# ygjwd12345/UCD

Measured on AMD Instinct MI355X. Metric: images/sec (whole node) per UCD train step, VOC 15-5 step-1, 513^2 bs=24, higher is better.
Workload: dtype bf16

## Files before the change

ucd_amd/csrc/stem.hip:

```cpp
#include "common.h"

namespace ucd {
namespace {

typedef __hip_bfloat16 bf16;
constexpr int kThreads = 256;
constexpr int kRedBlocks = 1024;
constexpr int kApplyRows = 4;

__device__ __forceinline__ float leaky(float z, float slope) { return z > 0.f ? z : z * slope; }
__device__ __forceinline__ float bf16_round(float v) { return __bfloat162float(__float2bfloat16(v)); }

struct StemArgs {
  const bf16* z; int B, H, W, C, PH, PW;
  const float *mean, *scale, *beta, *invstd, *weight, *sums;
  float slope, inv_count;
  int abs_gamma, cg_shift;
};

__global__ __launch_bounds__(kThreads) void stem_apply_pool_kernel(StemArgs p, bf16* __restrict__ out, uint8_t* __restrict__ idx) {
  const int cgs = p.cg_shift, CG = 1 << cgs;
  const int t = blockIdx.x * kThreads + threadIdx.x;
  const int cg = t & (CG - 1), pw = t >> cgs, ph = blockIdx.y, b = blockIdx.z;
  if (pw >= p.PW) return;
  const size_t pix = ((size_t)b * p.PH + ph) * p.PW + pw;
  float mu[8], sc[8], sh[8], best[8];
  int bi[8];
#pragma unroll
  for (int e = 0; e < 8; ++e) {
    mu[e] = p.mean[cg * 8 + e]; sc[e] = p.scale[cg * 8 + e]; sh[e] = p.beta ? p.beta[cg * 8 + e] : 0.f;
    best[e] = -INFINITY; bi[e] = 0;
  }
  Vec<bf16> v[9];
#pragma unroll
  for (int kh = 0; kh < 3; ++kh) {
    const int y = min(max(2 * ph - 1 + kh, 0), p.H - 1);
#pragma unroll
    for (int kw = 0; kw < 3; ++kw) {
      const int x = min(max(2 * pw - 1 + kw, 0), p.W - 1);
      v[kh * 3 + kw].load(p.z + (((size_t)b * p.H + y) * p.W + x) * p.C + cg * 8);
    }
  }
#pragma unroll
  for (int kh = 0; kh < 3; ++kh) {
    const bool yin = (unsigned)(2 * ph - 1 + kh) < (unsigned)p.H;
#pragma unroll
    for (int kw = 0; kw < 3; ++kw) {
      const bool in = yin && (unsigned)(2 * pw - 1 + kw) < (unsigned)p.W;
#pragma unroll
      for (int e = 0; e < 8; ++e) {
        const float a = bf16_round(leaky((v[kh * 3 + kw].get(e) - mu[e]) * sc[e] + sh[e], p.slope));
        if (in && a > best[e]) { best[e] = a; bi[e] = kh * 3 + kw; }
      }
    }
  }
  Vec<bf16> o;
#pragma unroll
  for (int e = 0; e < 8; ++e) o.set(e, best[e]);
  o.store(out + pix * p.C + cg * 8);
  if (idx) {
    uint2 w;
    w.x = (unsigned)bi[0] | ((unsigned)bi[1] << 8) | ((unsigned)bi[2] << 16) | ((unsigned)bi[3] << 24);
    w.y = (unsigned)bi[4] | ((unsigned)bi[5] << 8) | ((unsigned)bi[6] << 16) | ((unsigned)bi[7] << 24);
    *reinterpret_cast<uint2*>(idx + pix * p.C + cg * 8) = w;
  }
}

__global__ __launch_bounds__(kThreads) void stem_pool_bwd_reduce_kernel(StemArgs p, const bf16* __restrict__ dpool,
                                                                       const uint8_t* __restrict__ idx, float* __restrict__ partial) {
  extern __shared__ __attribute__((aligned(16))) float lds[];
  const int CG = p.C / 8, PL = kThreads / CG;
  const int cg = threadIdx.x % CG, pl = threadIdx.x / CG;
  const long long npix = (long long)p.B * p.PH * p.PW;
  float acc[16];
#pragma unroll
  for (int i = 0; i < 16; ++i) acc[i] = 0.f;
  if (pl < PL) {
    float mu[8], sc[8], sh[8], is[8];
#pragma unroll
    for (int e = 0; e < 8; ++e) {
      mu[e] = p.mean[cg * 8 + e]; sc[e] = p.scale[cg * 8 + e]; sh[e] = p.beta ? p.beta[cg * 8 + e] : 0.f; is[e] = p.invstd[cg * 8 + e];
    }
    for (int pix = blockIdx.x * PL + pl; pix < (int)npix; pix += gridDim.x * PL) {
      const int rowi = pix / p.PW;
      const int pw = pix - rowi * p.PW, b = rowi / p.PH, ph = rowi - b * p.PH;
      Vec<bf16> g;
      g.load(dpool + (size_t)pix * p.C + cg * 8);
      const uint2 w = *reinterpret_cast<const uint2*>(idx + (size_t)pix * p.C + cg * 8);
      float zsel[8] = {0.f, 0.f, 0.f, 0.f, 0.f, 0.f, 0.f, 0.f};
      Vec<bf16> v[9];
#pragma unroll
      for (int kh = 0; kh < 3; ++kh) {
        const int y = min(max(2 * ph - 1 + kh, 0), p.H - 1);
#pragma unroll
        for (int kw = 0; kw < 3; ++kw) {
          const int x = min(max(2 * pw - 1 + kw, 0), p.W - 1);
          v[kh * 3 + kw].load(p.z + (((size_t)b * p.H + y) * p.W + x) * p.C + cg * 8);
        }
      }
#pragma unroll
      for (int pos = 0; pos < 9; ++pos)
#pragma unroll
        for (int e = 0; e < 8; ++e) {
          const unsigned id = ((e < 4 ? w.x : w.y) >> (8 * (e & 3))) & 0xffu;
          zsel[e] = id == (unsigned)pos ? v[pos].get(e) : zsel[e];
        }
#pragma unroll
      for (int e = 0; e < 8; ++e) {
        const float xc = zsel[e] - mu[e];
        const float dz = g.get(e) * (xc * sc[e] + sh[e] > 0.f ? 1.f : p.slope);
        acc[e] += dz;
        acc[8 + e] += dz * (xc * is[e]);
      }
    }
  }
#pragma unroll
  for (int i = 0; i < 16; ++i) lds[threadIdx.x * 16 + i] = acc[i];
  __syncthreads();
  if (pl == 0) {
    for (int l = 1; l < PL; ++l)
#pragma unroll
      for (int i = 0; i < 16; ++i) acc[i] += lds[(l * CG + cg) * 16 + i];
    float* dst = partial + (size_t)blockIdx.x * 2 * p.C + cg * 8;
#pragma unroll
    for (int e = 0; e < 8; ++e) { dst[e] = acc[e]; dst[p.C + e] = acc[8 + e]; }
  }
}

__global__ __launch_bounds__(kThreads) void stem_pool_bwd_apply_kernel(StemArgs p, const bf16* __restrict__ dpool,
                                                                      const uint8_t* __restrict__ idx, bf16* __restrict__ dz) {
  const int cgs = p.cg_shift, CG = 1 << cgs;
  const int t = blockIdx.x * kThreads + threadIdx.x;
  const int cg = t & (CG - 1), i = t >> cgs, b = blockIdx.z;
  if (2 * i >= p.W) return;
  float mu[8], sc[8], sh[8], is[8], k0[8], k1[8], gw[8];
#pragma unroll
  for (int e = 0; e < 8; ++e) {
    const int ch = cg * 8 + e;
    mu[e] = p.mean[ch]; sc[e] = p.scale[ch]; sh[e] = p.beta ? p.beta[ch] : 0.f; is[e] = p.invstd[ch];
    k0[e] = p.sums[ch] * p.inv_count;
    k1[e] = p.sums[p.C + ch] * p.inv_count;
    if (p.abs_gamma) {
      if (p.weight && p.weight[ch] < 0.f) k1[e] = -k1[e];
      gw[e] = sc[e];
    } else {
      gw[e] = (p.weight ? p.weight[ch] : 1.f) * is[e];
    }
  }
  const int phb = blockIdx.y * 2, y0 = blockIdx.y * kApplyRows, x0 = 2 * i;
  Vec<bf16> g[3][2], v[kApplyRows][2];
  uint2 w[3][2];
  bool gv[3][2];
#pragma unroll
  for (int a = 0; a < 3; ++a)
#pragma unroll
    for (int c = 0; c < 2; ++c) {
      gv[a][c] = phb + a < p.PH && i + c < p.PW;
      const size_t off = (((size_t)b * p.PH + min(phb + a, p.PH - 1)) * p.PW + min(i + c, p.PW - 1)) * p.C + cg * 8;
      w[a][c] = *reinterpret_cast<const uint2*>(idx + off);
      g[a][c].load(dpool + off);
    }
#pragma unroll
  for (int r = 0; r < kApplyRows; ++r)
#pragma unroll
    for (int cx = 0; cx < 2; ++cx)
      v[r][cx].load(p.z + (((size_t)b * p.H + min(y0 + r, p.H - 1)) * p.W + min(x0 + cx, p.W - 1)) * p.C + cg * 8);
#pragma unroll
  for (int r = 0; r < kApplyRows; ++r) {
    if (y0 + r >= p.H) break;
#pragma unroll
    for (int cx = 0; cx < 2; ++cx) {
      if (x0 + cx >= p.W) continue;
      float dy[8] = {0.f, 0.f, 0.f, 0.f, 0.f, 0.f, 0.f, 0.f};
#pragma unroll
      for (int ya = 0; ya < 2; ++ya) {
        if (ya == 1 && !(r & 1)) continue;
        const int a = (r >> 1) + ya, kh = (r & 1) ? (ya ? 0 : 2) : 1;
#pragma unroll
        for (int xa = 0; xa < 2; ++xa) {
          if (xa == 1 && !cx) continue;
          const int kw = cx ? (xa ? 0 : 2) : 1;
          const unsigned pos = gv[a][xa] ? (unsigned)(kh * 3 + kw) : 0xffu;
#pragma unroll
          for (int e = 0; e < 8; ++e) {
            const unsigned id = ((e < 4 ? w[a][xa].x : w[a][xa].y) >> (8 * (e & 3))) & 0xffu;
            dy[e] += id == pos ? g[a][xa].get(e) : 0.f;
          }
        }
      }
      Vec<bf16> o;
#pragma unroll
      for (int e = 0; e < 8; ++e) {
        const float xc = v[r][cx].get(e) - mu[e];
        const float dza = dy[e] * (xc * sc[e] + sh[e] > 0.f ? 1.f : p.slope);
        o.set(e, (dza - k0[e] - (xc * is[e]) * k1[e]) * gw[e]);
      }
      o.store(dz + (((size_t)b * p.H + y0 + r) * p.W + x0 + cx) * p.C + cg * 8);
    }
  }
}

__global__ __launch_bounds__(kThreads) void stem_sum_partials_kernel(const float* __restrict__ partial, int rows, int C,
                                                                    const float* __restrict__ sign_of, float* __restrict__ sums) {
  __shared__ float red[kThreads];
  const int k = blockIdx.x;
  float s = 0.f;
  for (int r = threadIdx.x; r < rows; r += kThreads) s += partial[(size_t)r * 2 * C + k];
  red[threadIdx.x] = s;
  __syncthreads();
  for (int st = kThreads / 2; st > 0; st >>= 1) {
    if (threadIdx.x < st) red[threadIdx.x] += red[threadIdx.x + st];
    __syncthreads();
  }
  if (threadIdx.x == 0) {
    float t = red[0];
    if (sign_of && k >= C && sign_of[k - C] < 0.f) t = -t;
    sums[k] = t;
  }
}

constexpr int kSTH = 8, kSTW = 32;
constexpr int kSIR = 2 * kSTH + 5;
constexpr int kSIP = 216;
constexpr int kSWP = 184;
constexpr int kSK = 176;

struct StemConvArgs {
  const float* x; long long sb, sc, sh, sw;
  const bf16* w;
  bf16* z;
  int B, H, W, OH, OW, tiles_y, tiles_x, ntiles;
};

__global__ __launch_bounds__(kThreads) void stem_conv7x7_kernel(StemConvArgs p) {
  typedef float f32x16 __attribute__((ext_vector_type(16)));
  typedef __bf16 bf16x8 __attribute__((ext_vector_type(8)));
  __shared__ __attribute__((aligned(16))) unsigned short Wl[64 * kSWP];
  __shared__ __attribute__((aligned(16))) unsigned short In[kSIR * kSIP];
  const int tid = threadIdx.x, lane = tid & 63, wave = tid >> 6;
  for (int i = tid; i < 64 * kSWP; i += kThreads) Wl[i] = 0;
  __syncthreads();
  for (int i = tid; i < 64 * 147; i += kThreads) {
    const int n = i / 147, r = i - n * 147, ky = r / 21, j = r - ky * 21;
    Wl[n * kSWP + ky * 24 + j] = reinterpret_cast<const unsigned short*>(p.w)[i];
  }
  const int col = lane & 31, h = lane >> 5;
  const int fe = tid < kSIP ? tid : kSIP - 1, fpx = fe / 3, fc = fe - fpx * 3;
  float pre[kSIR];
  unsigned premask = 0;
  auto fetch = [&](int tile) {
    unsigned okm = 0;
    const int b = tile / (p.tiles_y * p.tiles_x), rem = tile - b * p.tiles_y * p.tiles_x;
    const int oy0 = (rem / p.tiles_x) * kSTH, ox0 = (rem % p.tiles_x) * kSTW;
    const int ix = 2 * ox0 - 3 + fpx;
    const bool colok = fpx < 2 * kSTW + 5 && (unsigned)ix < (unsigned)p.W;
    const float* src = p.x + b * p.sb + fc * p.sc + (colok ? ix : 0) * p.sw;
#pragma unroll
    for (int r = 0; r < kSIR; ++r) {
      const int iy = 2 * oy0 - 3 + r;
      const bool ok = colok && (unsigned)iy < (unsigned)p.H;
      const float v = src[(ok ? iy : 0) * p.sh];
      pre[r] = ok ? v : 0.f;
      okm |= 1u << r;
    }
    premask = okm;
  };
  if ((int)blockIdx.x < p.ntiles) fetch(blockIdx.x);
  for (int tile = blockIdx.x; tile < p.ntiles; tile += gridDim.x) {
    const int b = tile / (p.tiles_y * p.tiles_x), rem = tile - b * p.tiles_y * p.tiles_x;
    const int oy0 = (rem / p.tiles_x) * kSTH, ox0 = (rem % p.tiles_x) * kSTW;
    __syncthreads();
    if (tid < kSIP) {
#pragma unroll
      for (int r = 0; r < kSIR; ++r) {
        const bf16 v = __float2bfloat16((premask >> r) & 1u ? pre[r] : 0.f);
        In[r * kSIP + tid] = *reinterpret_cast<const unsigned short*>(&v);
      }
    }
    __syncthreads();
    if (tile + (int)gridDim.x < p.ntiles) fetch(tile + gridDim.x);
    f32x16 acc[2][2];
#pragma unroll
    for (int a = 0; a < 2; ++a)
#pragma unroll
      for (int c = 0; c < 2; ++c)
#pragma unroll
        for (int r = 0; r < 16; ++r) acc[a][c][r] = 0.f;
#pragma unroll
    for (int s = 0; s < kSK / 16; ++s) {
      const int t0 = 2 * s, t1 = 2 * s + 1;
      const int ky = h ? (t1 / 3 > 6 ? 6 : t1 / 3) : t0 / 3, j0 = h ? 8 * (t1 % 3) : 8 * (t0 % 3);
      bf16x8 wf[2], pf[2];
#pragma unroll
      for (int c = 0; c < 2; ++c) wf[c] = *reinterpret_cast<const bf16x8*>(&Wl[(c * 32 + col) * kSWP + 16 * s + 8 * h]);
#pragma unroll
      for (int a = 0; a < 2; ++a) {
        const int orow = wave * 2 + a;
        const unsigned* src = reinterpret_cast<const unsigned*>(&In[(2 * orow + ky) * kSIP + 6 * col + j0]);
        union { unsigned u[4]; bf16x8 v; } f;
        f.u[0] = src[0]; f.u[1] = src[1]; f.u[2] = src[2]; f.u[3] = src[3];
        pf[a] = f.v;
      }
#pragma unroll
      for (int a = 0; a < 2; ++a)
#pragma unroll
        for (int c = 0; c < 2; ++c) acc[a][c] = __builtin_amdgcn_mfma_f32_32x32x16_bf16(wf[c], pf[a], acc[a][c], 0, 0, 0);
    }
    const int ox = ox0 + col;
#pragma unroll
    for (int a = 0; a < 2; ++a) {
      const int oy = oy0 + wave * 2 + a;
      if (oy >= p.OH || ox >= p.OW) continue;
      bf16* dst = p.z + (((size_t)b * p.OH + oy) * p.OW + ox) * 64;
#pragma unroll
      for (int c = 0; c < 2; ++c)
#pragma unroll
        for (int g = 0; g < 4; ++g) {
          union { bf16 v[4]; uint2 u; } o;
#pragma unroll
          for (int e = 0; e < 4; ++e) o.v[e] = __float2bfloat16(acc[a][c][g * 4 + e]);
          *reinterpret_cast<uint2*>(dst + c * 32 + 8 * g + 4 * h) = o.u;
        }
    }
  }
}

constexpr int kFPH = 3, kFPW = 15;
constexpr int kFTP = 72;
struct StemFusedArgs {
  StemConvArgs c;
  const float *mean, *scale, *beta;
  float slope;
  bf16* out;
  int PH, PW;
};

__global__ __launch_bounds__(kThreads) void stem_conv_pool_kernel(StemFusedArgs q) {
  typedef float f32x16 __attribute__((ext_vector_type(16)));
  typedef __bf16 bf16x8 __attribute__((ext_vector_type(8)));
  const StemConvArgs& p = q.c;
  extern __shared__ __attribute__((aligned(16))) unsigned char fs_raw[];
  unsigned short* Wl = reinterpret_cast<unsigned short*>(fs_raw);
  unsigned short* In = Wl + 64 * kSWP;
  unsigned short* Tl = In + kSIR * kSIP;
  float* Pl = reinterpret_cast<float*>(Tl + kSTH * kSTW * kFTP);
  const int tid = threadIdx.x, lane = tid & 63, wave = tid >> 6;
  for (int i = tid; i < 64 * kSWP; i += kThreads) Wl[i] = 0;
  if (tid < 64) { Pl[tid] = q.mean[tid]; Pl[64 + tid] = q.scale[tid]; Pl[128 + tid] = q.beta ? q.beta[tid] : 0.f; }
  __syncthreads();
  for (int i = tid; i < 64 * 147; i += kThreads) {
    const int n = i / 147, r = i - n * 147, ky = r / 21, j = r - ky * 21;
    Wl[n * kSWP + ky * 24 + j] = reinterpret_cast<const unsigned short*>(p.w)[i];
  }
  const int col = lane & 31, h = lane >> 5;
  const int fe = tid < kSIP ? tid : kSIP - 1, fpx = fe / 3, fc = fe - fpx * 3;
  float pre[kSIR];
  unsigned premask = 0;
  auto origin = [&](int tile, int& b, int& oy0, int& ox0) {
    b = tile / (p.tiles_y * p.tiles_x);
    const int rem = tile - b * p.tiles_y * p.tiles_x;
    oy0 = 2 * (rem / p.tiles_x) * kFPH - 1;
    ox0 = 2 * (rem % p.tiles_x) * kFPW - 1;
  };
  auto fetch = [&](int tile) {
    unsigned okm = 0;
    int b, oy0, ox0;
    origin(tile, b, oy0, ox0);
    const int ix = 2 * ox0 - 3 + fpx;
    const bool colok = fpx < 2 * kSTW + 5 && (unsigned)ix < (unsigned)p.W;
    const float* src = p.x + b * p.sb + fc * p.sc + (colok ? ix : 0) * p.sw;
#pragma unroll
    for (int r = 0; r < kSIR; ++r) {
      const int iy = 2 * oy0 - 3 + r;
      const bool ok = colok && (unsigned)iy < (unsigned)p.H;
      pre[r] = src[(ok ? iy : 0) * p.sh];
      okm |= ok ? (1u << r) : 0u;
    }
    premask = okm;
  };
  if ((int)blockIdx.x < p.ntiles) fetch(blockIdx.x);
  for (int tile = blockIdx.x; tile < p.ntiles; tile += gridDim.x) {
    int b, oy0, ox0;
    origin(tile, b, oy0, ox0);
    __syncthreads();
    if (tid < kSIP) {
#pragma unroll
      for (int r = 0; r < kSIR; ++r) {
        const bf16 v = __float2bfloat16((premask >> r) & 1u ? pre[r] : 0.f);
        In[r * kSIP + tid] = *reinterpret_cast<const unsigned short*>(&v);
      }
    }
    __syncthreads();
    if (tile + (int)gridDim.x < p.ntiles) fetch(tile + gridDim.x);
    f32x16 acc[2][2];
#pragma unroll
    for (int a = 0; a < 2; ++a)
#pragma unroll
      for (int c = 0; c < 2; ++c)
#pragma unroll
        for (int r = 0; r < 16; ++r) acc[a][c][r] = 0.f;
#pragma unroll
    for (int s = 0; s < kSK / 16; ++s) {
      const int t0 = 2 * s, t1 = 2 * s + 1;
      const int ky = h ? (t1 / 3 > 6 ? 6 : t1 / 3) : t0 / 3, j0 = h ? 8 * (t1 % 3) : 8 * (t0 % 3);
      bf16x8 wf[2], pf[2];
#pragma unroll
      for (int c = 0; c < 2; ++c) wf[c] = *reinterpret_cast<const bf16x8*>(&Wl[(c * 32 + col) * kSWP + 16 * s + 8 * h]);
#pragma unroll
      for (int a = 0; a < 2; ++a) {
        const int orow = wave * 2 + a;
        const unsigned* src = reinterpret_cast<const unsigned*>(&In[(2 * orow + ky) * kSIP + 6 * col + j0]);
        union { unsigned u[4]; bf16x8 v; } f;
        f.u[0] = src[0]; f.u[1] = src[1]; f.u[2] = src[2]; f.u[3] = src[3];
        pf[a] = f.v;
      }
#pragma unroll
      for (int a = 0; a < 2; ++a)
#pragma unroll
        for (int c = 0; c < 2; ++c) acc[a][c] = __builtin_amdgcn_mfma_f32_32x32x16_bf16(wf[c], pf[a], acc[a][c], 0, 0, 0);
    }
    const int ox = ox0 + col;
#pragma unroll
    for (int a = 0; a < 2; ++a) {
      const int orow = wave * 2 + a, oy = oy0 + orow;
      const bool inside = (unsigned)oy < (unsigned)p.OH && (unsigned)ox < (unsigned)p.OW;
      unsigned short* dst = Tl + (orow * kSTW + col) * kFTP;
#pragma unroll
      for (int c = 0; c < 2; ++c)
#pragma unroll
        for (int g = 0; g < 4; ++g) {
          const int ch = c * 32 + 8 * g + 4 * h;
          const float4 mu = *reinterpret_cast<const float4*>(Pl + ch), sc = *reinterpret_cast<const float4*>(Pl + 64 + ch);
          const float4 sh = *reinterpret_cast<const float4*>(Pl + 128 + ch);
          const float m4[4] = {mu.x, mu.y, mu.z, mu.w}, s4[4] = {sc.x, sc.y, sc.z, sc.w}, b4[4] = {sh.x, sh.y, sh.z, sh.w};
          union { bf16 v[4]; uint2 u; } o;
#pragma unroll
          for (int e = 0; e < 4; ++e) {
            const float zq = bf16_round(acc[a][c][g * 4 + e]);
            o.v[e] = __float2bfloat16(leaky((zq - m4[e]) * s4[e] + b4[e], q.slope));
          }
          if (!inside) o.u = make_uint2(0xFF80FF80u, 0xFF80FF80u);
          *reinterpret_cast<uint2*>(dst + ch) = o.u;
        }
    }
    __syncthreads();
    for (int i = tid; i < kFPH * kFPW * 8; i += kThreads) {
      const int cg = i & 7, pp = i >> 3, pr = pp / kFPW, pc = pp - pr * kFPW;
      const int ph = (oy0 + 1) / 2 + pr, pw = (ox0 + 1) / 2 + pc;
      if (ph >= q.PH || pw >= q.PW) continue;
      float best[8];
#pragma unroll
      for (int e = 0; e < 8; ++e) best[e] = -INFINITY;
#pragma unroll
      for (int kh = 0; kh < 3; ++kh)
#pragma unroll
        for (int kw = 0; kw < 3; ++kw) {
          Vec<bf16> v;
          v.raw = *reinterpret_cast<const uint4*>(Tl + ((2 * pr + kh) * kSTW + 2 * pc + kw) * kFTP + cg * 8);
#pragma unroll
          for (int e = 0; e < 8; ++e) best[e] = fmaxf(best[e], v.get(e));
        }
      Vec<bf16> o;
#pragma unroll
      for (int e = 0; e < 8; ++e) o.set(e, best[e]);
      o.store(q.out + (((size_t)b * q.PH + ph) * q.PW + pw) * 64 + cg * 8);
    }
  }
}

bool stem_args_ok(const void* z, int B, int H, int W, int C) {
  return z && B > 0 && B < 65536 && H > 1 && H < 65536 && W > 1 && C >= 8 && (C & (C - 1)) == 0 && C <= 2048 && aligned16(z);
}

}
}

using namespace ucd;

extern "C" {

int ucd_stem_pooled_size(int n) { return (n + 2 - 3) / 2 + 1; }

size_t ucd_stem_pool_workspace_bytes(int C) { return (size_t)kRedBlocks * 2 * C * sizeof(float); }

int ucd_stem_apply_pool(const void* z, int B, int H, int W, int C, const float* mean, const float* scale, const float* beta, int act,
                        float slope, void* out, uint8_t* idx, ucd_stream_t stream) {
  static const char* fn = "ucd_stem_apply_pool";
  UCD_REQUIRE(stem_args_ok(z, B, H, W, C) && mean && scale && out && aligned16(out) && (!idx || (reinterpret_cast<uintptr_t>(idx) & 7) == 0),
              UCD_EINVAL, "%s: dense channels-last bf16 maps with a power-of-two channel count in 8..2048 expected", fn);
  const int a = act & UCD_ACT_MASK;
  UCD_REQUIRE(a != UCD_ACT_ELU, UCD_EUNSUPPORTED, "%s: leaky_relu / identity only (an elu stem keeps the separate passes)", fn);
  StemArgs p{};
  p.z = (const bf16*)z; p.B = B; p.H = H; p.W = W; p.C = C; p.PH = ucd_stem_pooled_size(H); p.PW = ucd_stem_pooled_size(W);
  p.mean = mean; p.scale = scale; p.beta = beta; p.slope = a == UCD_ACT_IDENTITY ? 1.f : slope;
  p.cg_shift = __builtin_ctz(C / 8);
  stem_apply_pool_kernel<<<dim3(ceil_div(p.PW * (C / 8), kThreads), p.PH, B), kThreads, 0, (hipStream_t)stream>>>(p, (bf16*)out, idx);
  return check_launch(fn);
}

int ucd_stem_conv7x7(const float* x, long long sb, long long sc, long long sh, long long sw, int B, int H, int W, const void* w,
                     void* z, ucd_stream_t stream) {
  static const char* fn = "ucd_stem_conv7x7";
  UCD_REQUIRE(x && w && z && B > 0 && H > 0 && W > 0 && aligned16(z) && (reinterpret_cast<uintptr_t>(w) & 1) == 0, UCD_EINVAL,
              "%s: bad arguments", fn);
  StemConvArgs p{};
  p.x = x; p.sb = sb; p.sc = sc; p.sh = sh; p.sw = sw; p.w = (const bf16*)w; p.z = (bf16*)z;
  p.B = B; p.H = H; p.W = W; p.OH = (H + 6 - 7) / 2 + 1; p.OW = (W + 6 - 7) / 2 + 1;
  p.tiles_y = ceil_div(p.OH, kSTH); p.tiles_x = ceil_div(p.OW, kSTW); p.ntiles = B * p.tiles_y * p.tiles_x;
  const int grid = p.ntiles < 768 ? p.ntiles : 768;
  stem_conv7x7_kernel<<<grid, kThreads, 0, (hipStream_t)stream>>>(p);
  return check_launch(fn);
}

int ucd_stem_conv_pool(const float* x, long long sb, long long sc, long long sh, long long sw, int B, int H, int W, const void* w,
                       const float* mean, const float* scale, const float* beta, int act, float slope, void* out, ucd_stream_t stream) {
  static const char* fn = "ucd_stem_conv_pool";
  UCD_REQUIRE(x && w && out && mean && scale && B > 0 && H > 0 && W > 0 && aligned16(out) && (reinterpret_cast<uintptr_t>(w) & 1) == 0 &&
              aligned16(mean) && aligned16(scale) && (!beta || aligned16(beta)), UCD_EINVAL, "%s: bad arguments", fn);
  const int a = act & UCD_ACT_MASK;
  UCD_REQUIRE(a != UCD_ACT_ELU && !(act & UCD_NORM_ABS_GAMMA), UCD_EUNSUPPORTED, "%s: leaky_relu / identity with given scale only", fn);
  StemFusedArgs q{};
  StemConvArgs& p = q.c;
  p.x = x; p.sb = sb; p.sc = sc; p.sh = sh; p.sw = sw; p.w = (const bf16*)w; p.z = nullptr;
  p.B = B; p.H = H; p.W = W; p.OH = (H + 6 - 7) / 2 + 1; p.OW = (W + 6 - 7) / 2 + 1;
  q.PH = ucd_stem_pooled_size(p.OH); q.PW = ucd_stem_pooled_size(p.OW);
  p.tiles_y = ceil_div(q.PH, kFPH); p.tiles_x = ceil_div(q.PW, kFPW); p.ntiles = B * p.tiles_y * p.tiles_x;
  q.mean = mean; q.scale = scale; q.beta = beta; q.slope = a == UCD_ACT_IDENTITY ? 1.f : slope; q.out = (bf16*)out;
  const size_t lds = (size_t)(64 * kSWP + kSIR * kSIP + kSTH * kSTW * kFTP) * 2 + 3 * 64 * 4;
  UCD_TRY_LDS(stem_conv_pool_kernel, 80 * 1024);
  const int grid = p.ntiles < 512 ? p.ntiles : 512;
  stem_conv_pool_kernel<<<grid, kThreads, lds, (hipStream_t)stream>>>(q);
  return check_launch(fn);
}

int ucd_stem_pool_backward(const void* z, const void* dpool, const uint8_t* idx, int B, int H, int W, int C, const float* mean,
                           const float* invstd, const float* scale, const float* beta, const float* weight, float* sums, float count,
                           int act, float slope, void* dz, void* workspace, size_t workspace_bytes, int phase, ucd_stream_t stream) {
  static const char* fn = "ucd_stem_pool_backward";
  UCD_REQUIRE(stem_args_ok(z, B, H, W, C) && dpool && idx && mean && invstd && scale && sums && aligned16(dpool), UCD_EINVAL,
              "%s: bad arguments", fn);
  UCD_REQUIRE(phase >= 1 && phase <= 3 && (!(phase & 2) || (dz && aligned16(dz) && count > 0.f)), UCD_EINVAL, "%s: bad phase / dz", fn);
  const int a = act & UCD_ACT_MASK;
  UCD_REQUIRE(a != UCD_ACT_ELU, UCD_EUNSUPPORTED, "%s: leaky_relu / identity only", fn);
  StemArgs p{};
  p.z = (const bf16*)z; p.B = B; p.H = H; p.W = W; p.C = C; p.PH = ucd_stem_pooled_size(H); p.PW = ucd_stem_pooled_size(W);
  p.mean = mean; p.scale = scale; p.beta = beta; p.invstd = invstd; p.weight = weight; p.sums = sums;
  p.slope = a == UCD_ACT_IDENTITY ? 1.f : slope; p.abs_gamma = (act & UCD_NORM_ABS_GAMMA) != 0;
  p.cg_shift = __builtin_ctz(C / 8);
  hipStream_t s = (hipStream_t)stream;
  if (phase & 1) {
    UCD_REQUIRE(workspace && workspace_bytes >= ucd_stem_pool_workspace_bytes(C), UCD_EWORKSPACE, "%s: workspace too small", fn);
    stem_pool_bwd_reduce_kernel<<<kRedBlocks, kThreads, kThreads * 16 * sizeof(float), s>>>(p, (const bf16*)dpool, idx, (float*)workspace);
    int rc = check_launch(fn);
    if (rc) return rc;
    stem_sum_partials_kernel<<<2 * C, kThreads, 0, s>>>((const float*)workspace, kRedBlocks, C, p.abs_gamma ? weight : nullptr, sums);
    rc = check_launch(fn);
    if (rc) return rc;
  }
  if (phase & 2) {
    p.inv_count = 1.f / count;
    stem_pool_bwd_apply_kernel<<<dim3(ceil_div(((W + 1) / 2) * (C / 8), kThreads), ceil_div(H, kApplyRows), B), kThreads, 0, s>>>(p, (const bf16*)dpool, idx, (bf16*)dz);
    return check_launch(fn);
  }
  return 0;
}

}
```

Measured before the change: 846.7.

## Tile stem BN-act-maxpool over 2x2 outputs, gather-only backward, packed math

Measured after the change: 849.3, median of 6. About the same (+0.3%).

```diff
diff --git a/ucd_amd/csrc/stem.hip b/ucd_amd/csrc/stem.hip
--- a/ucd_amd/csrc/stem.hip
+++ b/ucd_amd/csrc/stem.hip
@@ -18,102 +18,154 @@
   int abs_gamma, cg_shift;
 };
 
-__global__ __launch_bounds__(kThreads) void stem_apply_pool_kernel(StemArgs p, bf16* __restrict__ out, uint8_t* __restrict__ idx) {
+constexpr int kPoolRows = 2, kPoolCols = 2;
+constexpr int kZRows = 2 * kPoolRows + 1, kZCols = 2 * kPoolCols + 1;
+
+template <bool MAXACT>
+__global__ __launch_bounds__(kThreads) void stem_apply_pool_kernel(StemArgs p, int strips, int cgroups, bf16* __restrict__ out,
+                                                                  uint8_t* __restrict__ idx) {
   const int cgs = p.cg_shift, CG = 1 << cgs;
   const int t = blockIdx.x * kThreads + threadIdx.x;
-  const int cg = t & (CG - 1), pw = t >> cgs, ph = blockIdx.y, b = blockIdx.z;
-  if (pw >= p.PW) return;
-  const size_t pix = ((size_t)b * p.PH + ph) * p.PW + pw;
-  float mu[8], sc[8], sh[8], best[8];
-  int bi[8];
-#pragma unroll
-  for (int e = 0; e < 8; ++e) {
-    mu[e] = p.mean[cg * 8 + e]; sc[e] = p.scale[cg * 8 + e]; sh[e] = p.beta ? p.beta[cg * 8 + e] : 0.f;
-    best[e] = -INFINITY; bi[e] = 0;
-  }
-  Vec<bf16> v[9];
-#pragma unroll
-  for (int kh = 0; kh < 3; ++kh) {
-    const int y = min(max(2 * ph - 1 + kh, 0), p.H - 1);
-#pragma unroll
-    for (int kw = 0; kw < 3; ++kw) {
-      const int x = min(max(2 * pw - 1 + kw, 0), p.W - 1);
-      v[kh * 3 + kw].load(p.z + (((size_t)b * p.H + y) * p.W + x) * p.C + cg * 8);
-    }
-  }
-#pragma unroll
-  for (int kh = 0; kh < 3; ++kh) {
-    const bool yin = (unsigned)(2 * ph - 1 + kh) < (unsigned)p.H;
-#pragma unroll
-    for (int kw = 0; kw < 3; ++kw) {
-      const bool in = yin && (unsigned)(2 * pw - 1 + kw) < (unsigned)p.W;
+  const int cg = t & (CG - 1), q = t >> cgs, b = blockIdx.y;
+  if (q >= strips * cgroups) return;
+  const int strip = q / cgroups, ph0 = strip * kPoolRows, pw0 = (q - strip * cgroups) * kPoolCols;
+  const int y0 = 2 * ph0 - 1, x0 = 2 * pw0 - 1;
+  const Pack8 mu = load_pairs<4>(p.mean + cg * 8), sc = load_pairs<4>(p.scale + cg * 8);
+  const Pack8 sh = p.beta ? load_pairs<4>(p.beta + cg * 8) : zero_pairs<4>();
+  const int csh = cgs + 3;
+  const bf16* zb = p.z + ((size_t)b * p.H * p.W << csh) + cg * 8;
+  uint4 v[kZRows][kZCols];
+#pragma unroll
+  for (int r = 0; r < kZRows; ++r) {
+    const unsigned yw = (unsigned)min(max(y0 + r, 0), p.H - 1) * p.W;
+#pragma unroll
+    for (int c = 0; c < kZCols; ++c) {
+      const int x = min(max(x0 + c, 0), p.W - 1);
+      v[r][c] = *reinterpret_cast<const uint4*>(zb + ((size_t)(yw + x) << csh));
+    }
+  }
+  uint32_t xin[kZCols];
+#pragma unroll
+  for (int c = 0; c < kZCols; ++c) xin[c] = (unsigned)(x0 + c) < (unsigned)p.W ? 0xFFFFFFFFu : 0u;
+  float best[kPoolRows][kPoolCols][8];
+  unsigned bi[kPoolRows][kPoolCols][8];
+#pragma unroll
+  for (int r = 0; r < kZRows; ++r) {
+    const uint32_t yin = (unsigned)(y0 + r) < (unsigned)p.H ? 0xFFFFFFFFu : 0u;
+    float a[kZCols][8];
+#pragma unroll
+    for (int c = 0; c < kZCols; ++c) {
+      const Pack8 x = unpack8(v[r][c]);
+#pragma unroll
+      for (int j = 0; j < 4; ++j) {
+        const f32x2 t = (x.p[j] - mu.p[j]) * sc.p[j] + sh.p[j], ts = t * p.slope;
+        const f32x2 y = MAXACT ? f32x2{__builtin_fmaxf(t.x, ts.x), __builtin_fmaxf(t.y, ts.y)} : leaky2(t, p.slope);
+        uint32_t w = __builtin_bit_cast(uint32_t, __builtin_convertvector(y, bf16x2v));
+        w = (w & (yin & xin[c])) | (0xFF80FF80u & ~(yin & xin[c]));
+        a[c][2 * j] = __uint_as_float(w << 16);
+        a[c][2 * j + 1] = __uint_as_float(w & 0xFFFF0000u);
+      }
+    }
+#pragma unroll
+    for (int k = 0; k < kPoolCols; ++k)
 #pragma unroll
       for (int e = 0; e < 8; ++e) {
-        const float a = bf16_round(leaky((v[kh * 3 + kw].get(e) - mu[e]) * sc[e] + sh[e], p.slope));
-        if (in && a > best[e]) { best[e] = a; bi[e] = kh * 3 + kw; }
-      }
-    }
-  }
-  Vec<bf16> o;
-#pragma unroll
-  for (int e = 0; e < 8; ++e) o.set(e, best[e]);
-  o.store(out + pix * p.C + cg * 8);
-  if (idx) {
-    uint2 w;
-    w.x = (unsigned)bi[0] | ((unsigned)bi[1] << 8) | ((unsigned)bi[2] << 16) | ((unsigned)bi[3] << 24);
-    w.y = (unsigned)bi[4] | ((unsigned)bi[5] << 8) | ((unsigned)bi[6] << 16) | ((unsigned)bi[7] << 24);
-    *reinterpret_cast<uint2*>(idx + pix * p.C + cg * 8) = w;
-  }
-}
-
+        float m = -INFINITY;
+        unsigned kw = 0;
+#pragma unroll
+        for (int c = 0; c < 3; ++c)
+          if (a[2 * k + c][e] > m) { m = a[2 * k + c][e]; kw = c; }
+        if (r & 1) {
+          if (m > best[r / 2][k][e]) { best[r / 2][k][e] = m; bi[r / 2][k][e] = 3 + kw; }
+        } else {
+          if (r >= 2 && m > best[r / 2 - 1][k][e]) { best[r / 2 - 1][k][e] = m; bi[r / 2 - 1][k][e] = 6 + kw; }
+          if (r / 2 < kPoolRows) { best[r / 2][k][e] = m; bi[r / 2][k][e] = kw; }
+        }
+      }
+  }
+#pragma unroll
+  for (int i = 0; i < kPoolRows; ++i) {
+    if (ph0 + i >= p.PH) break;
+#pragma unroll
+    for (int k = 0; k < kPoolCols; ++k) {
+      if (pw0 + k >= p.PW) continue;
+      const size_t pix = (size_t)b * p.PH * p.PW + (unsigned)(ph0 + i) * p.PW + pw0 + k;
+      Pack8 o;
+#pragma unroll
+      for (int j = 0; j < 4; ++j) o.p[j] = f32x2{best[i][k][2 * j], best[i][k][2 * j + 1]};
+      *reinterpret_cast<uint4*>(out + (pix << csh) + cg * 8) = pack8(o);
+      if (idx) {
+        const unsigned* n = bi[i][k];
+        uint2 w;
+        w.x = n[0] | (n[1] << 8) | (n[2] << 16) | (n[3] << 24);
+        w.y = n[4] | (n[5] << 8) | (n[6] << 16) | (n[7] << 24);
+        *reinterpret_cast<uint2*>(idx + (pix << csh) + cg * 8) = w;
+      }
+    }
+  }
+}
+
+struct StemPoolReq { uint4 g; uint2 w; };
 __global__ __launch_bounds__(kThreads) void stem_pool_bwd_reduce_kernel(StemArgs p, const bf16* __restrict__ dpool,
                                                                        const uint8_t* __restrict__ idx, float* __restrict__ partial) {
   extern __shared__ __attribute__((aligned(16))) float lds[];
   const int CG = p.C / 8, PL = kThreads / CG;
   const int cg = threadIdx.x % CG, pl = threadIdx.x / CG;
-  const long long npix = (long long)p.B * p.PH * p.PW;
-  float acc[16];
-#pragma unroll
-  for (int i = 0; i < 16; ++i) acc[i] = 0.f;
+  const int npix = p.B * p.PH * p.PW;
+  f32x2 s1[4], s2[4];
+#pragma unroll
+  for (int j = 0; j < 4; ++j) { s1[j] = f32x2{0.f, 0.f}; s2[j] = f32x2{0.f, 0.f}; }
   if (pl < PL) {
-    float mu[8], sc[8], sh[8], is[8];
-#pragma unroll
-    for (int e = 0; e < 8; ++e) {
-      mu[e] = p.mean[cg * 8 + e]; sc[e] = p.scale[cg * 8 + e]; sh[e] = p.beta ? p.beta[cg * 8 + e] : 0.f; is[e] = p.invstd[cg * 8 + e];
-    }
-    for (int pix = blockIdx.x * PL + pl; pix < (int)npix; pix += gridDim.x * PL) {
+    const Pack8 mu = load_pairs<4>(p.mean + cg * 8), sc = load_pairs<4>(p.scale + cg * 8), is = load_pairs<4>(p.invstd + cg * 8);
+    const Pack8 sh = p.beta ? load_pairs<4>(p.beta + cg * 8) : zero_pairs<4>();
+    const int step = gridDim.x * PL, row_elems = p.W * p.C;
+    auto request = [&](int pix, StemPoolReq& q) {
+      const size_t off = (size_t)min(pix, npix - 1) * p.C + cg * 8;
+      q.g = *reinterpret_cast<const uint4*>(dpool + off);
+      q.w = *reinterpret_cast<const uint2*>(idx + off);
+    };
+    auto gather = [&](int pix, const uint2& w, unsigned short (&zr)[8]) {
+      pix = min(pix, npix - 1);
       const int rowi = pix / p.PW;
       const int pw = pix - rowi * p.PW, b = rowi / p.PH, ph = rowi - b * p.PH;
-      Vec<bf16> g;
-      g.load(dpool + (size_t)pix * p.C + cg * 8);
-      const uint2 w = *reinterpret_cast<const uint2*>(idx + (size_t)pix * p.C + cg * 8);
-      float zsel[8] = {0.f, 0.f, 0.f, 0.f, 0.f, 0.f, 0.f, 0.f};
-      Vec<bf16> v[9];
-#pragma unroll
-      for (int kh = 0; kh < 3; ++kh) {
-        const int y = min(max(2 * ph - 1 + kh, 0), p.H - 1);
-#pragma unroll
-        for (int kw = 0; kw < 3; ++kw) {
-          const int x = min(max(2 * pw - 1 + kw, 0), p.W - 1);
-          v[kh * 3 + kw].load(p.z + (((size_t)b * p.H + y) * p.W + x) * p.C + cg * 8);
-        }
-      }
-#pragma unroll
-      for (int pos = 0; pos < 9; ++pos)
-#pragma unroll
-        for (int e = 0; e < 8; ++e) {
-          const unsigned id = ((e < 4 ? w.x : w.y) >> (8 * (e & 3))) & 0xffu;
-          zsel[e] = id == (unsigned)pos ? v[pos].get(e) : zsel[e];
-        }
+      const bf16* org = p.z + (((long long)b * p.H + 2 * ph - 1) * p.W + 2 * pw - 1) * p.C + cg * 8;
+      const int kh_lo = ph == 0 ? 1 : 0, kh_hi = min(2, p.H - 2 * ph), kw_lo = pw == 0 ? 1 : 0, kw_hi = min(2, p.W - 2 * pw);
 #pragma unroll
       for (int e = 0; e < 8; ++e) {
-        const float xc = zsel[e] - mu[e];
-        const float dz = g.get(e) * (xc * sc[e] + sh[e] > 0.f ? 1.f : p.slope);
-        acc[e] += dz;
-        acc[8 + e] += dz * (xc * is[e]);
-      }
-    }
-  }
+        const int id = ((e < 4 ? w.x : w.y) >> (8 * (e & 3))) & 0xffu;
+        const int kh3 = (id * 11) >> 5;
+        const int kh = min(max(kh3, kh_lo), kh_hi), kw = min(max(id - 3 * kh3, kw_lo), kw_hi);
+        zr[e] = *reinterpret_cast<const unsigned short*>(org + (kh * row_elems + kw * p.C + e));
+      }
+    };
+    int pix = blockIdx.x * PL + pl;
+    StemPoolReq q0, q1;
+    unsigned short za[8];
+    request(pix, q0);
+    request(pix + step, q1);
+    gather(pix, q0.w, za);
+    for (; pix < npix; pix += step) {
+      unsigned short zb[8];
+      StemPoolReq q2;
+      gather(pix + step, q1.w, zb);
+      request(pix + 2 * step, q2);
+      const Pack8 g = unpack8(q0.g);
+#pragma unroll
+      for (int j = 0; j < 4; ++j) {
+        const f32x2 zs = f32x2{__uint_as_float((uint32_t)za[2 * j] << 16), __uint_as_float((uint32_t)za[2 * j + 1] << 16)};
+        const f32x2 xc = zs - mu.p[j];
+        const f32x2 dz = leaky_grad2(g.p[j], xc * sc.p[j] + sh.p[j], p.slope);
+        s1[j] += dz;
+        s2[j] += dz * (xc * is.p[j]);
+      }
+      q0 = q1; q1 = q2;
+#pragma unroll
+      for (int e = 0; e < 8; ++e) za[e] = zb[e];
+    }
+  }
+  float acc[16];
+#pragma unroll
+  for (int j = 0; j < 4; ++j) { acc[2 * j] = s1[j].x; acc[2 * j + 1] = s1[j].y; acc[8 + 2 * j] = s2[j].x; acc[8 + 2 * j + 1] = s2[j].y; }
 #pragma unroll
   for (int i = 0; i < 16; ++i) lds[threadIdx.x * 16 + i] = acc[i];
   __syncthreads();
@@ -133,20 +185,10 @@
   const int t = blockIdx.x * kThreads + threadIdx.x;
   const int cg = t & (CG - 1), i = t >> cgs, b = blockIdx.z;
   if (2 * i >= p.W) return;
-  float mu[8], sc[8], sh[8], is[8], k0[8], k1[8], gw[8];
-#pragma unroll
-  for (int e = 0; e < 8; ++e) {
-    const int ch = cg * 8 + e;
-    mu[e] = p.mean[ch]; sc[e] = p.scale[ch]; sh[e] = p.beta ? p.beta[ch] : 0.f; is[e] = p.invstd[ch];
-    k0[e] = p.sums[ch] * p.inv_count;
-    k1[e] = p.sums[p.C + ch] * p.inv_count;
-    if (p.abs_gamma) {
-      if (p.weight && p.weight[ch] < 0.f) k1[e] = -k1[e];
-      gw[e] = sc[e];
-    } else {
-      gw[e] = (p.weight ? p.weight[ch] : 1.f) * is[e];
-    }
-  }
+  const int c0 = cg * 8;
+  const Pack8 mu = load_pairs<4>(p.mean + c0), sc = load_pairs<4>(p.scale + c0), is = load_pairs<4>(p.invstd + c0);
+  const Pack8 a0 = load_pairs<4>(p.sums + c0), a1 = load_pairs<4>(p.sums + p.C + c0);
+  const Pack8 shl = load_pairs<4>((p.beta ? p.beta : p.mean) + c0), wl = load_pairs<4>((p.weight ? p.weight : p.mean) + c0);
   const int phb = blockIdx.y * 2, y0 = blockIdx.y * kApplyRows, x0 = 2 * i;
   Vec<bf16> g[3][2], v[kApplyRows][2];
   uint2 w[3][2];
@@ -165,13 +207,32 @@
 #pragma unroll
     for (int cx = 0; cx < 2; ++cx)
       v[r][cx].load(p.z + (((size_t)b * p.H + min(y0 + r, p.H - 1)) * p.W + min(x0 + cx, p.W - 1)) * p.C + cg * 8);
+  const bool has_beta = p.beta != nullptr, has_weight = p.weight != nullptr;
+  Pack8 sh, k0, k1, gw, gq[3][2];
+#pragma unroll
+  for (int j = 0; j < 4; ++j) {
+    sh.p[j] = has_beta ? shl.p[j] : f32x2{0.f, 0.f};
+    k0.p[j] = a0.p[j] * p.inv_count;
+    k1.p[j] = a1.p[j] * p.inv_count;
+    if (p.abs_gamma) {
+      const f32x2 n = -k1.p[j];
+      if (has_weight) k1.p[j] = f32x2{wl.p[j].x < 0.f ? n.x : k1.p[j].x, wl.p[j].y < 0.f ? n.y : k1.p[j].y};
+      gw.p[j] = sc.p[j];
+    } else {
+      gw.p[j] = (has_weight ? wl.p[j] : f32x2{1.f, 1.f}) * is.p[j];
+    }
+  }
+#pragma unroll
+  for (int a = 0; a < 3; ++a)
+#pragma unroll
+    for (int c = 0; c < 2; ++c) gq[a][c] = unpack8(g[a][c].raw);
 #pragma unroll
   for (int r = 0; r < kApplyRows; ++r) {
     if (y0 + r >= p.H) break;
 #pragma unroll
     for (int cx = 0; cx < 2; ++cx) {
       if (x0 + cx >= p.W) continue;
-      float dy[8] = {0.f, 0.f, 0.f, 0.f, 0.f, 0.f, 0.f, 0.f};
+      Pack8 dy = zero_pairs<4>();
 #pragma unroll
       for (int ya = 0; ya < 2; ++ya) {
         if (ya == 1 && !(r & 1)) continue;
@@ -182,20 +243,21 @@
           const int kw = cx ? (xa ? 0 : 2) : 1;
           const unsigned pos = gv[a][xa] ? (unsigned)(kh * 3 + kw) : 0xffu;
 #pragma unroll
-          for (int e = 0; e < 8; ++e) {
-            const unsigned id = ((e < 4 ? w[a][xa].x : w[a][xa].y) >> (8 * (e & 3))) & 0xffu;
-            dy[e] += id == pos ? g[a][xa].get(e) : 0.f;
+          for (int j = 0; j < 4; ++j) {
+            const unsigned ids = (j < 2 ? w[a][xa].x : w[a][xa].y) >> (16 * (j & 1));
+            dy.p[j] += f32x2{(ids & 0xffu) == pos ? gq[a][xa].p[j].x : 0.f, ((ids >> 8) & 0xffu) == pos ? gq[a][xa].p[j].y : 0.f};
           }
         }
       }
-      Vec<bf16> o;
-#pragma unroll
-      for (int e = 0; e < 8; ++e) {
-        const float xc = v[r][cx].get(e) - mu[e];
-        const float dza = dy[e] * (xc * sc[e] + sh[e] > 0.f ? 1.f : p.slope);
-        o.set(e, (dza - k0[e] - (xc * is[e]) * k1[e]) * gw[e]);
-      }
-      o.store(dz + (((size_t)b * p.H + y0 + r) * p.W + x0 + cx) * p.C + cg * 8);
+      const Pack8 x = unpack8(v[r][cx].raw);
+      Pack8 o;
+#pragma unroll
+      for (int j = 0; j < 4; ++j) {
+        const f32x2 xc = x.p[j] - mu.p[j];
+        const f32x2 dza = leaky_grad2(dy.p[j], xc * sc.p[j] + sh.p[j], p.slope);
+        o.p[j] = (dza - k0.p[j] - (xc * is.p[j]) * k1.p[j]) * gw.p[j];
+      }
+      *reinterpret_cast<uint4*>(dz + (((size_t)b * p.H + y0 + r) * p.W + x0 + cx) * p.C + cg * 8) = pack8(o);
     }
   }
 }
@@ -469,7 +531,7 @@
 }
 
 bool stem_args_ok(const void* z, int B, int H, int W, int C) {
-  return z && B > 0 && B < 65536 && H > 1 && H < 65536 && W > 1 && C >= 8 && (C & (C - 1)) == 0 && C <= 2048 && aligned16(z);
+  return z && B > 0 && B < 65536 && H > 1 && H < 65536 && W > 1 && W < 65536 && C >= 8 && (C & (C - 1)) == 0 && C <= 2048 && aligned16(z);
 }
 
 }
@@ -494,7 +556,10 @@
   p.z = (const bf16*)z; p.B = B; p.H = H; p.W = W; p.C = C; p.PH = ucd_stem_pooled_size(H); p.PW = ucd_stem_pooled_size(W);
   p.mean = mean; p.scale = scale; p.beta = beta; p.slope = a == UCD_ACT_IDENTITY ? 1.f : slope;
   p.cg_shift = __builtin_ctz(C / 8);
-  stem_apply_pool_kernel<<<dim3(ceil_div(p.PW * (C / 8), kThreads), p.PH, B), kThreads, 0, (hipStream_t)stream>>>(p, (bf16*)out, idx);
+  const int strips = ceil_div(p.PH, kPoolRows), cgroups = ceil_div(p.PW, kPoolCols);
+  const dim3 grid(ceil_div(strips * cgroups * (C / 8), kThreads), B);
+  if (p.slope > 0.f && p.slope <= 1.f) stem_apply_pool_kernel<true><<<grid, kThreads, 0, (hipStream_t)stream>>>(p, strips, cgroups, (bf16*)out, idx);
+  else stem_apply_pool_kernel<false><<<grid, kThreads, 0, (hipStream_t)stream>>>(p, strips, cgroups, (bf16*)out, idx);
   return check_launch(fn);
 }
 
```
